# gruai/koifish

Measured on AMD Instinct MI355X. Metric: tokens/sec/GPU Qwen3 4-bit prefill+decode; achieved HBM GB/s vs peak, higher is better.
Workload: dtype u4 weights x bf16, fp32 accumulate

## Files before the change

koifish_amd/csrc/kf_abi.hip:

```cpp
#include <stdarg.h>
#include <stdio.h>
#include <string.h>


#include <mutex>
#include <math.h>
#include <stdlib.h>

#include <vector>

#include "kf_gemm_plan.h"

struct kf_ctx {
    int device;
    hipStream_t stream;
    bool own_stream;
    bool capturing;
    float* amax_val;
    int* amax_idx;
    int canonical;
    void* scratch;
    size_t scratch_bytes;
    struct DeqCopy {
        const void* key[3];
// ... 1246 lines not shown
    if (rc != KF_OK) return fail(rc, "kf_xengine_check: HIP failure");
    if (err) return fail(KF_INTERNAL_ERR, "kf_xengine: error word 0x%x (8: an XCD did not get 32 workgroups; 64: a position beyond the cache rows (TP form); others: a hand-off poll timed out -- the launch was not fully resident)", err);
    return KF_OK;
}
int kf_xengine_reset(kf_ctx* c, kf_xengine* e) {
    CHKCTX(c);
    if (!e || !e->h) return fail(KF_INVALID_ARGS, "kf_xengine_reset: null engine");
    if (c->capturing) return fail(KF_INVALID_ARGS, "kf_xengine_reset: not while capturing");
    if (hipStreamSynchronize(c->stream) != hipSuccess) return fail(KF_HIP_CHECK, "kf_xengine_reset: HIP failure");
    const int rc = kf::xengine_reset(e->h, c->stream);
    if (rc != KF_OK) return fail(rc, "kf_xengine_reset: HIP failure");
    return KF_OK;
}
int kf_xengine_destroy(kf_xengine* e) {
    if (e) {
        kf::xengine_free(e->h);
        delete e;
    }
    return KF_OK;
}
int kfdbg_xengine_variant(kf_xengine* e, int nwv, int depth) { return (e && e->h) ? kf::xengine_set_variant(e->h, nwv, depth) : -1; }
int kfdbg_xengine_form(int shape_class, int fmt, int n_seq, int n_layer, int stamps, int two_wpc, int* out) {
    const kf::XForm* f = kf::xengine_form(shape_class, fmt, n_seq, n_layer, stamps != 0, two_wpc != 0);
    if (!f || !out) return -1;
    out[0] = f->nwv, out[1] = f->depth, out[2] = f->wpc, out[3] = f->nb, out[4] = f->dbg;
    return 0;
}
int kfdbg_engine_form(int shape_class, int fmt, int canon, int stamps, int n_layer, int* out) {
    const kf::EngForm* f = kf::engine_form(shape_class, fmt, canon != 0, stamps != 0, n_layer);
    if (!f || !out) return -1;
    out[0] = f->shape_class, out[1] = f->fmt, out[2] = f->canon, out[3] = f->dbg, out[4] = (int)f->smem(n_layer);
    return 0;
}
int kfdbg_xengine_stamps_enable(kf_xengine* e, int seq, int wg, int max_steps) { return (e && e->h) ? kf::xengine_debug_enable(e->h, seq, wg, max_steps) : -1; }
int kfdbg_xengine_stamps(kf_xengine* e, unsigned long long* h_out, int n_words) { return (e && e->h) ? kf::xengine_debug_read(e->h, h_out, n_words) : -1; }
int kfdbg_engine_stamps_enable(kf_engine* e, int wg) { return (e && e->h) ? kf::engine_debug_enable(e->h, wg) : -1; }
int kfdbg_engine_stamps(kf_engine* e, unsigned long long* h_out, int n_words) { return (e && e->h) ? kf::engine_debug_read(e->h, h_out, n_words) : -1; }
int kfdbg_engine_set_delays(kf_engine* e, const int* d6) {
    if (!e || !e->h || !d6) return -1;
    kf::engine_set_delays(e->h, d6);
    return 0;
}
int kfdbg_gemm_plan(const kf::GemmProblem* P, kf::GemmPlan* out) {
    if (!P || !out) return -1;
    *out = kf::gemm_plan(*P);
    return 0;
}
int kfdbg_set_knob(const char* name, long value) {
    if (!name) return -1;
    kf::Knobs& k = kf::g_knobs;
    if (!strcmp(name, "q4_perm")) k.q4_perm = (int)value;
    else if (!strcmp(name, "q2_tab")) k.q2_tab = (int)value;
    else if (!strcmp(name, "q1_tab")) k.q1_tab = (int)value;
    else if (!strcmp(name, "gemv_waves")) k.gemv_waves = value;
    else if (!strcmp(name, "gemv_stream")) k.gemv_stream = (int)value;
    else if (!strcmp(name, "gemv_xf2")) k.gemv_xf2 = (int)value;
    else if (!strcmp(name, "attn_gq_split")) k.attn_gq_split = (int)value;
    else if (!strcmp(name, "attn_pair_min")) k.attn_pair_min = (int)value;
    else return -1;
    return 0;
}
int kf_engine_destroy(kf_engine* e) {
    if (e) {
        kf::engine_free(e->h);
        delete e;
    }
// ... 5 lines not shown
```

koifish_amd/csrc/kf_engine.hip:

```cpp
#include <stdlib.h>
#include <string.h>

#include <vector>

#include <type_traits>

#include "kf_engine_common.h"

namespace kf {


struct EngXOff {
    int xA, qkv, ao, xB, act, part, hbest, tokg, end;
};
constexpr EngXOff eng_xoff(int dim, int qd, int kvd, int ffn, int hd) {
    EngXOff o{};
    o.xA = 0, o.qkv = o.xA + eng_gran_dw(dim), o.ao = o.qkv + eng_gran_dw(qd + 2 * kvd), o.xB = o.ao + eng_gran_dw(qd), o.act = o.xB + eng_gran_dw(dim);
    o.part = o.act + eng_gran_dw(ffn);
    o.hbest = o.part + eng_gran_dw(2 * (qd / hd) * KF_ATTN_MAX_SPLITS * (2 * hd + 4));
    o.tokg = o.hbest + eng_gran_dw(2 * ENG_NWG);
    o.end = o.tokg + eng_gran_dw(2);
    return o;
}
constexpr int eng_lq_stride(int gq, int hd) { return ((gq * hd + 2 * hd) * 4 + 255) / 256 * 64; }
constexpr int eng_lp_stride(int gq, int hd) { return (gq * KF_ATTN_MAX_SPLITS * (2 * hd + 4) * 8 + 255) / 256 * 32; }
constexpr size_t eng_loc_bytes(int gq, int hd) { return 1024 + (size_t)8 * eng_lq_stride(gq, hd) * 4 + (size_t)8 * eng_lp_stride(gq, hd) * 8; }

struct EngArgs {
    const EngLayer* layers;
    int n_layer;
    int n_steps;
    float eps, qk_eps;
    const float* rope_table;
    const int32_t* d_state;
    const uint16_t* x_in;
    const uint16_t* emb;
    const int32_t* d_forced;
    int emb_rows;
    uint16_t* x_out;
    uint32_t* xch;
    int* ws;
    char* loc;
    int nsp, chunk, merge_e;
    int kv_stride;
    int max_seq;
    float qbias[7];
    int delay[6];
    g_u32x4 head_w;
    g_u16 head_norm;
    uint16_t* logits;
    int32_t* d_state_w;
// ... 20 lines not shown
        for (int i = 0; i < NR; i++) {
            const int r = wave + i * NWV;
            g[i] = __builtin_bit_cast(u32x4, __builtin_amdgcn_raw_buffer_load_b128(rs, ((r < NLD ? r : wave) * 64 + lane) * 16, 0, 16 ));
        }
#pragma unroll
        for (int i = 0; i < NR; i++) bad = (wave + i * NWV < NLD) ? tags_bad(g[i], tagw, bad) : bad;
        if (wave >= NLD || all_good(bad)) {
            if (nsweeps) *nsweeps = spins + 1;
            break;
        }
        if (dead || spins > ENG_SPIN_MAX) {
            if (!dead && lane == 0) atomicOr(ws + 1, 1);
            dead = true;
            break;
        }
        __builtin_amdgcn_s_sleep(1);
    }
#pragma unroll
    for (int i = 0; i < NR; i++) {
        const int r = wave + i * NWV;
        if (r >= NLD) continue;
        const int e0 = 4 * (r * 64 + lane);
        const uint32_t o0 = (g[i].x & 0xffffu) | (g[i].y << 16), o1 = (g[i].z & 0xffffu) | (g[i].w << 16);
        if (F32X) {
            const int q = e0 >> 2, c = q / XCH, j = q - c * XCH;
            xs[j * NBLK + c] = u32x4{o0 << 16, o0 & 0xffff0000u, o1 << 16, o1 & 0xffff0000u};
        } else {
            const int q = e0 >> 3, c = q / XCH, j = q - c * XCH;
            reinterpret_cast<u32x2*>(xs + j * NBLK + c)[(e0 >> 2) & 1] = u32x2{o0, o1};
        }
    }
}

template <bool PAIRED, int MAXS>
struct MvRegs {
    u32x4 w[MAXS], w2[PAIRED ? MAXS : 1];
    uint16_t st[MAXS], ze[MAXS], st2[PAIRED ? MAXS : 1], ze2[PAIRED ? MAXS : 1];
};
template <class PL, int NCW>
constexpr int c_maxs() { return ((PL::spg + NCW - 1) / NCW) * PL::iters; }
template <class PL, int NCW>
__device__ __forceinline__ MvAt mv_at(int k, int s0, int cw, int lane, int Mj) {
    const int sub = lane >> PL::lpr_log2, ll = lane & (PL::LPR - 1);
    const int sl = k / PL::iters, it = k - sl * PL::iters;
    const int s_loc = cw + sl * NCW;
    MvAt q;
    q.row = (s0 + s_loc) * PL::RPS + sub;
    q.col = it * PL::LPR + ll;
    q.ok = s_loc < PL::spg && q.row < Mj && q.col < PL::nBlk;
    return q;
}
template <class PL, int NCW, int FMT, int MAXS>
__device__ __forceinline__ void mv_prefetch(const EngMat m, const EngMat m2, int s0, int cw, int lane, int Mj, MvRegs<PL::PAIRED, MAXS>& R, uint32_t hotbits = 0xffffffffu) {
    constexpr bool GAMA = BlockDot<FMT>::HAS_GAMA;
    constexpr int gshift = FMT >= FMT_Q4 ? (FMT == FMT_Q4 || FMT == FMT_Q4P || FMT == FMT_Q1T || FMT == FMT_Q2T ? 2 : (FMT == FMT_Q2 ? 1 : 0)) : 0;
#pragma unroll
    for (int k = 0; k < MAXS; k++) {
        const MvAt q = mv_at<PL, NCW>(k, s0, cw, lane, Mj);
        int row = q.row < Mj ? q.row : Mj - 1;
        row = row > 0 ? row : 0;
        row = ((hotbits >> ((q.row - s0 * PL::RPS) & 31)) & 1u) ? row : 0;
        const int col = q.col < PL::nBlk ? q.col : PL::nBlk - 1;
        const uint32_t bidx = (uint32_t)row * (uint32_t)PL::nBlk + (uint32_t)col;
        if constexpr (FMT == FMT_Q1T) {
            const uint32_t di = (bidx & ~3u) + (3u - (bidx & 3u));
            R.w[k] = u32x4{__builtin_nontemporal_load(reinterpret_cast<const uint32_t KF_GLOBAL*>(m.w) + di), 0u, 0u, 0u};
// ... 120 lines not shown
    double* comb;
    uint32_t* outb;
    int* cnt;
    double* msc;
    int* pub;
    const u32x4* q1tab;
    const uint32_t* hotbits;
};
struct EngSlice {
    int pos, len, nsp, kvh, split, h0, t0, t1, me0;
    bool has_unit, empty, own_new, has_merge;
    int xcc, rank;
    int j1;
    int s1;
    int M1;
    int q_out0;
};

__device__ __forceinline__ void wg_publish(const EngLds& L, int phase, uint32_t* buf, int idx0, int nrows, int nwaves, int lane, bool local = false) {
    int old = 0;
    if (lane == 0) old = __hip_atomic_fetch_add(L.cnt, 1, __ATOMIC_RELAXED, __HIP_MEMORY_SCOPE_WORKGROUP);
    old = __builtin_amdgcn_readfirstlane(old);
    if (old != nwaves - 1) return;
    if (lane == 0) *L.cnt = 0;
    if (4 * lane < nrows) {
        const u32x4 v = *reinterpret_cast<const u32x4*>(L.outb + 4 * lane);
        if (local)
            *reinterpret_cast<u32x4*>(buf + idx0 + 4 * lane) = v;
        else
            __builtin_amdgcn_raw_buffer_store_b128(v, eng_rsrc(buf + idx0, (uint32_t)nrows * 4u), lane * 16, 0, 16 );
    }
    if (lane == 0) __hip_atomic_fetch_add(L.pub + phase, 1, __ATOMIC_RELAXED, __HIP_MEMORY_SCOPE_WORKGROUP);
}

template <int FMT_, int GQ_, int HD_, int NWV_, int DIM_, int QD_, int KVD_, int FFN_, int NWG_, bool XMAP_, bool DBG_, bool CANON_ = true>
struct EngCfg {
    static constexpr int FMT = FMT_, GQ = GQ_, HD = HD_, NWV = NWV_, DIM = DIM_, QD = QD_, KVD = KVD_, FFN = FFN_, NWG = NWG_;
    static constexpr bool XMAP = XMAP_, DBG = DBG_;
    static constexpr int AHR = DIM_ > 1024 ? ENG_AH_REGS_WIDE : ENG_AH_REGS;
    static constexpr int AHR_P = DIM_ > 1024 ? ENG_AH_PAIR_WIDE : ENG_AH_REGS;
    static constexpr bool CANON = CANON_;
    static_assert(FMT_ == FMT_Q4 || FMT_ == FMT_Q4P || FMT_ == FMT_Q1T || FMT_ == FMT_Q2T, "storages with a BlockPrep: 32-weight blocks dequantised ahead of the hand-off (16 pair words each)");
    static constexpr bool F32X = CANON_;
    static constexpr int XCH = F32X ? 8 : 4;
    static constexpr int n_head = QD_ / HD_, n_kv = KVD_ / HD_;
    using SH = EngShape<FMT_, DIM_, QD_, KVD_, FFN_, NWG_>;
    static constexpr int xA = eng_xoff(DIM_, QD_, KVD_, FFN_, HD_).xA, qkv = eng_xoff(DIM_, QD_, KVD_, FFN_, HD_).qkv, ao = eng_xoff(DIM_, QD_, KVD_, FFN_, HD_).ao,
                         xB = eng_xoff(DIM_, QD_, KVD_, FFN_, HD_).xB, act = eng_xoff(DIM_, QD_, KVD_, FFN_, HD_).act, part = eng_xoff(DIM_, QD_, KVD_, FFN_, HD_).part,
                         hbest = eng_xoff(DIM_, QD_, KVD_, FFN_, HD_).hbest, tokg = eng_xoff(DIM_, QD_, KVD_, FFN_, HD_).tokg;
    static constexpr int HnBlk = DIM_ / 8, Hlpr_log2 = c_lpr_log2(DIM_ / 8, 1L << 20), HLPR = 1 << Hlpr_log2, HRPS = 64 >> Hlpr_log2, Hiters = (HnBlk + HLPR - 1) / HLPR;
    static constexpr int lq_stride = eng_lq_stride(GQ_, HD_), lp_stride = eng_lp_stride(GQ_, HD_);
    static constexpr int ME = pow2_ceil((QD_ + NWG_ - 1) / NWG_), PSH = KF_ATTN_MAX_SPLITS * (2 * HD_ + 4), NLM = (KF_ATTN_MAX_SPLITS * ME * 2 + 127) / 128;
    static_assert(ME <= 64 && ME <= HD_, "merge elements per workgroup");
};
template <class C>
__device__ __forceinline__ uint32_t* eng_lqkv(const EngArgs& a, int xcc) { return reinterpret_cast<uint32_t*>(a.loc + 1024) + (size_t)xcc * C::lq_stride; }
template <class C>
__device__ __forceinline__ unsigned long long* eng_lpart(const EngArgs& a, int xcc) {
    return reinterpret_cast<unsigned long long*>(a.loc + 1024 + (size_t)8 * C::lq_stride * 4) + (size_t)xcc * C::lp_stride;
}

template <class C>
struct EngAttnState {
    static constexpr int U = 2;
    u32x4 kk[U], vv[U];
    uint16_t nw0, nw1;
    float rc, rs;
};
template <class C>
__device__ __forceinline__ void eng_attn_rope(const EngArgs& a, const EngSlice& S, int lane, EngAttnState<C>& T) {
    T.rc = 1.f, T.rs = 0.f;
    if (a.rope_table && lane < (C::HD >> 1)) {
        const float* tab_pos = a.rope_table + (size_t)S.pos * C::HD;
        T.rc = tab_pos[2 * lane], T.rs = tab_pos[2 * lane + 1];
    }
}
template <class C>
__device__ __forceinline__ void eng_attn_normw(const EngLayer& ly, int wave, int lane, EngAttnState<C>& T) {
    const int half = C::HD >> 1, j = lane < half ? lane : half - 1;
    static_assert(C::GQ < C::NWV, "the q heads and the new key are prepared by different waves");
    g_u16 np = wave < C::GQ ? ly.norm_q : ly.norm_k;
    T.nw0 = T.nw1 = 0;
// ... 142 lines not shown
                    st_gran64(dst + oi, gen, __uint_as_float((uint32_t)ob)), st_gran64(dst + oi + 1, gen, __uint_as_float((uint32_t)(ob >> 32)));
                    if (d == 0) st_gran64(dst + mi, gen, ms), st_gran64(dst + mi + 1, gen, __uint_as_float((uint32_t)lb)), st_gran64(dst + mi + 2, gen, __uint_as_float((uint32_t)(lb >> 32)));
                }
            }
        }
    } else if (nsp > 1) {
        for (int i = tid; i < GQ * hd; i += NWA * 64) {
            const int hq = i >> hd_log2, d = i & (hd - 1);
            constexpr int ME = C::ME, MAXSP = KF_ATTN_MAX_SPLITS;
            const size_t oi = ((size_t)(d / ME) * (MAXSP * ME) + (size_t)S.split * ME + (d & (ME - 1))) * 2, mi = (size_t)hd * MAXSP * 2 + (size_t)S.split * 4;
            const unsigned long long gg = (unsigned long long)gen << 32;
            if (XMAP) {
                unsigned long long* dst = eng_lpart<C>(a, S.xcc) + (size_t)hq * C::PSH;
                dst[oi] = gg, dst[oi + 1] = gg;
                if (d == 0) dst[mi] = gg | 0xff800000u, dst[mi + 1] = gg, dst[mi + 2] = gg;
            } else {
                unsigned long long* dst = reinterpret_cast<unsigned long long*>(a.xch + C::part) + (size_t)(h0 + hq) * C::PSH;
                st_gran64(dst + oi, gen, 0.f), st_gran64(dst + oi + 1, gen, 0.f);
                if (d == 0) st_gran64(dst + mi, gen, -__builtin_inff()), st_gran64(dst + mi + 1, gen, 0.f), st_gran64(dst + mi + 2, gen, 0.f);
            }
        }
    }
}

template <class C>
__device__ __forceinline__ void eng_poller_main(const EngArgs& a, const EngLds& L, const EngSlice& S, int epoch, int step, int wg, int lane) {
    using SH = typename C::SH;
    using P1 = typename SH::P1;
    using P4 = typename SH::P4;
    using P5 = typename SH::P5;
    using P6 = typename SH::P6;
    constexpr int FMT = C::FMT, GQ = C::GQ, HD = C::HD, NWV = C::NWV;
    constexpr bool XMAP = C::XMAP, DBG = C::DBG;
    constexpr int ND = C::DIM / 256, NQD = C::QD / 256, NF = C::FFN / 256;
    constexpr int XCH = C::XCH, hd = HD, hd_log2 = HD == 128 ? 7 : 6;
    bool dead = false;
    const bool has1 = XMAP ? true : wg * P1::spg < P1::total, has4 = wg * P4::spg < P4::total, has5 = wg * P5::spg < P5::total, has6 = wg * P6::spg < P6::total;
    constexpr int NCW1 = ENG_P1_SHARE ? NWV : NWV - 1, S1 = c_maxs<P1, NCW1>(), NWP1 = P1::spg < NCW1 ? P1::spg : NCW1;
    constexpr bool P1_SHARE = ENG_P1_SHARE && P1::spg >= NWV;
    const float qb1 = S.j1 == 0 ? a.qbias[0] : (S.j1 == 1 ? a.qbias[1] : a.qbias[2]);
    const int row0_1 = S.s1 * P1::RPS;
    MvRegs<false, S1> r1;
    auto mat1 = [&](int l) {
        return L.lay[l].m[S.j1];
    };
    if (P1_SHARE) mv_prefetch<P1, NCW1, FMT, S1>(mat1(0), mat1(0), S.s1, NWV - 1, lane, S.M1, r1);
    EngAttnState<C> T;
#pragma unroll
    for (int u = 0; u < EngAttnState<C>::U; u++) T.kk[u] = T.vv[u] = u32x4{0, 0, 0, 0};
    eng_attn_rope<C>(a, S, lane, T);
    if (S.has_unit && !S.empty) eng_attn_issue<C>(a, L.lay[0], S, NWV - 1, lane, T, 0);
    int sw[4] = {0, 0, 0, 0};
    int swt[6] = {0, 0, 0, 0, 0, 0};
    for (int l = 0; l < a.n_layer; l++) {
        const EngLayer& ly = L.lay[l];
        const uint32_t gen = (uint32_t)epoch * (uint32_t)a.n_layer + (uint32_t)l, tag = gen & 0xffffu;
        if (S.has_unit && !S.empty) eng_attn_normw<C>(ly, NWV - 1, lane, T);
        MvPhase<C, P1, NCW1, S1> w1;
        if (P1_SHARE) w1.ahead(qb1, 0.f, NWV - 1, lane, r1, L.q1tab);
        ENG_STAMP(0, 0);
        if (has1 || has4) {
            if (l == 0) {
                const uint16_t* x0 = a.x_in;
                if (!x0) {
                    int tok = a.d_state[0];
                    if (step > 0) {
                        const __amdgpu_buffer_rsrc_t rt = eng_rsrc(a.xch + C::tokg, 8u);
// ... 145 lines not shown
                    for (int k = 0; k < MAXSP; k++) o += ldexp_d(mv[k], shl[k]);
                }
            }
            const uint32_t gr = (tag << 16) | (uint32_t)f2bf((float)(o / Lt));
            const bool holder = (4 * ME <= 64) ? ((lane & 3) == 0 && (lane >> 2) < ME) : (lane < ME);
            const int he = (4 * ME <= 64) ? (lane >> 2) : lane;
            uint32_t* const ao_dst = a.xch + C::ao + (XMAP ? S.h0 * hd : 0) + S.me0;
            if (ME >= 4) {
                uint32_t* mo = reinterpret_cast<uint32_t*>(L.msc + ME * MAXSP);
                if (holder) mo[he] = gr;
                if (4 * lane < ME) __builtin_amdgcn_raw_buffer_store_b128(*reinterpret_cast<const u32x4*>(mo + 4 * lane), eng_rsrc(ao_dst, (uint32_t)ME * 4u), lane * 16, 0, 16 );
            } else if (holder) {
                __hip_atomic_store(ao_dst + he, gr, __ATOMIC_RELAXED, __HIP_MEMORY_SCOPE_AGENT);
            }
        }
        ENG_STAMP(0, 4);
        if (ENG_COOP) {
            if (has4) eng_wait_pub(nullptr, 0, a.delay[3], dead);
            __syncthreads();
            if (has4) eng_poll_stage_part<XCH, NQD, P4::nBlk, NWV, C::F32X>(a.xch + C::ao, tag, L.xs[1], NWV - 1, lane, a.ws, dead, &sw[1]);
        } else if (has4) {
            eng_poll_stage<XCH, NQD, P4::nBlk, false, false, C::F32X>(a.xch + C::ao, nullptr, tag, nullptr, 0.f, L.xs[1], nullptr, lane, a.ws, dead, &sw[1], nullptr, 0, a.delay[3]);
        }
        ENG_STAMP(0, 5);
        __syncthreads();
        if (has5 || has6)
            eng_poll_stage<XCH, ND, P5::nBlk, true, false, C::F32X>(a.xch + C::xB, nullptr, tag, ly.norm_post, a.eps, L.xs[0], L.xrawB, lane, a.ws, dead, &sw[2], has4 ? L.pub + 1 : nullptr, l + 1,
                                                           a.delay[4]);
        ENG_STAMP(0, 6);
        __syncthreads();
        if (ENG_COOP) {
            if (has6) eng_wait_pub(has5 ? L.pub + 2 : nullptr, l + 1, a.delay[5], dead);
            __syncthreads();
            if (has6) eng_poll_stage_part<XCH, NF, P6::nBlk, NWV, C::F32X>(a.xch + C::act, tag, L.xs[1], NWV - 1, lane, a.ws, dead, &sw[3]);
        } else if (has6) {
            eng_poll_stage<XCH, NF, P6::nBlk, false, false, C::F32X>(a.xch + C::act, nullptr, tag, nullptr, 0.f, L.xs[1], nullptr, lane, a.ws, dead, &sw[3], has5 ? L.pub + 2 : nullptr, l + 1, a.delay[5]);
        }
        ENG_STAMP(0, 7);
        swt[0] += sw[0], swt[3] += sw[1], swt[4] += sw[2], swt[5] += sw[3];
        if (DBG && wg == a.dbg_wg && lane == 0)
            a.dbg[((size_t)l * 2) * 16 + 8] = (unsigned long long)sw[0] | ((unsigned long long)sw[1] << 16) | ((unsigned long long)sw[2] << 32) | ((unsigned long long)sw[3] << 48);
        __syncthreads();
    }
    if (wg == 0 && lane == 0) {
#pragma unroll
        for (int i = 0; i < 6; i++) atomicAdd(a.ws + 8 + i, swt[i]);
        atomicAdd(a.ws + 14, a.n_layer);
    }
}

template <class C>
__device__ __forceinline__ void eng_compute_main(const EngArgs& a, const EngLds& L, const EngSlice& S, int epoch, int wg, int wave, int lane) {
    using SH = typename C::SH;
    using P1 = typename SH::P1;
    using P4 = typename SH::P4;
    using P5 = typename SH::P5;
    using P6 = typename SH::P6;
    constexpr int FMT = C::FMT, NWV = C::NWV;
    constexpr bool XMAP = C::XMAP, DBG = C::DBG;
    constexpr int NCW = NWV - 1;
    constexpr int NCW1 = ENG_P1_SHARE ? NWV : NWV - 1;
    constexpr int S1 = c_maxs<P1, NCW1>(), S4 = c_maxs<P4, NCW>(), S5 = c_maxs<P5, NCW>(), S6 = c_maxs<P6, NCW>();
    static_assert(P1::R % 4 == 0 && P4::R % 4 == 0 && P5::R % 4 == 0 && P6::R % 4 == 0 && P1::R <= 64 && P4::R <= 64 && P5::R <= 64 && P6::R <= 64, "rows per workgroup");
    static_assert(P1::total % P1::spg == 0 && P4::total % P4::spg == 0 && P5::total % P5::spg == 0 && P6::total % P6::spg == 0, "whole workgroups");
    static_assert(P1::S1 % P1::spg == 0 && P1::S2 % P1::spg == 0, "a workgroup's P1 rows belong to one matrix");
    constexpr int NWP1 = P1::spg < NCW1 ? P1::spg : NCW1, NWP4 = P4::spg < NCW ? P4::spg : NCW, NWP5 = P5::spg < NCW ? P5::spg : NCW, NWP6 = P6::spg < NCW ? P6::spg : NCW;
    const bool has1 = XMAP ? true : wg * P1::spg < P1::total, has4 = wg * P4::spg < P4::total, has5 = wg * P5::spg < P5::total, has6 = wg * P6::spg < P6::total;
    const float qb1 = S.j1 == 0 ? a.qbias[0] : (S.j1 == 1 ? a.qbias[1] : a.qbias[2]);
    const int row0_1 = S.s1 * P1::RPS;
// ... 41 lines not shown
            const int lane_a = lane + lz;
            eng_attn_phase<C>(a, L, S, ly, gen, tag, wave, lane_a, T, l, wg);
            if (wave == 0) ENG_STAMP(1, 3);
            if (DBG && wave == 0) {
                asm volatile("s_waitcnt vmcnt(0)" ::: "memory");
                ENG_STAMP(1, 10);
            }
            if (!S.empty) eng_attn_issue<C>(a, L.lay[ln], S, wave, lane_a, T, 0);
        }

        MvPhase<C, P4, NCW, S4> w4;
        w4.ahead(a.qbias[3], 0.f, wave, lane_m, r4, L.q1tab);
        if (ENG_COOP) {
            __syncthreads();
            if (has4) eng_poll_stage_part<C::XCH, C::QD / 256, P4::nBlk, NWV, C::F32X>(a.xch + C::ao, tag, L.xs[1], wave, lane_m, a.ws, dead);
        }
        __syncthreads();
        if (wave == 0) ENG_STAMP(1, 4);
        const uint32_t hot5 = L.hotbits[l];
        mv_prefetch<P5, NCW, FMT, S5>(ly.m[4], ly.m[5], wg * P5::spg, wave, lane_m, P5::M0, r5, hot5);
        w4.run(wg * P4::spg, wave, lane_m, P4::M0, L.xs[1], 0xffffffffu, r4, [&](int row, float v, float) {
            const uint16_t o = f2bf(v);
            L.outb[row - wg * P4::R] = (tag << 16) | (uint32_t)f2bf(bf2f(L.xrawA[row]) + bf2f(o));
        });
        if (has4 && wave < NWP4) wg_publish(L, 1, a.xch + C::xB, wg * P4::R, P4::R, NWP4, lane_m);
        if (wave == 0) ENG_STAMP(1, 5);
        MvPhase<C, P5, NCW, S5> w5;
        w5.ahead(a.qbias[4], a.qbias[5], wave, lane_m, r5, L.q1tab);
        __syncthreads();
        if (wave == 0) ENG_STAMP(1, 6);
        mv_prefetch<P6, NCW, FMT, S6>(ly.m[6], ly.m[6], wg * P6::spg, wave, lane_m, P6::M0, r6);
        w5.run(wg * P5::spg, wave, lane_m, P5::M0, L.xs[0], L.hotbits[l], r5, [&](int row, float v, float v2) {
            const float gt = round_bf16(v), up = round_bf16(v2);
            L.outb[row - wg * P5::R] = (tag << 16) | (uint32_t)f2bf((gt * up) / (1.0f + kf_expf(-gt)));
        });
        if (has5 && wave < NWP5) wg_publish(L, 2, a.xch + C::act, wg * P5::R, P5::R, NWP5, lane_m);
        if (wave == 0) ENG_STAMP(1, 7);
        MvPhase<C, P6, NCW, S6> w6;
        w6.ahead(a.qbias[6], 0.f, wave, lane_m, r6, L.q1tab);
        if (ENG_COOP) {
            __syncthreads();
            if (has6) eng_poll_stage_part<C::XCH, C::FFN / 256, P6::nBlk, NWV, C::F32X>(a.xch + C::act, tag, L.xs[1], wave, lane_m, a.ws, dead);
        }
        __syncthreads();
        if (wave == 0) ENG_STAMP(1, 8);
        mv_prefetch<P1, NCW1, FMT, S1>(mat1(ln), mat1(ln), S.s1, wave, lane_m, S.M1, r1);
        w6.run(wg * P6::spg, wave, lane_m, P6::M0, L.xs[1], 0xffffffffu, r6, [&](int row, float v, float) {
            const uint16_t o = f2bf(v);
            const uint16_t y = f2bf(bf2f(L.xrawB[row]) + bf2f(o));
            if (last) a.x_out[row] = y;
            L.outb[row - wg * P6::R] = (tag_next << 16) | (uint32_t)y;
        });
        if ((!last || a.head_on) && has6 && wave < NWP6) wg_publish(L, 3, a.xch + C::xA, wg * P6::R, P6::R, NWP6, lane_m);
        if (wave == 0) ENG_STAMP(1, 9);
    }
}


template <class C>
__device__ __forceinline__ void eng_head_main(const EngArgs& a, const EngLds& L, int epoch, bool more_steps, int wg, int wave, int lane) {
    constexpr int NWV = C::NWV, NWG = C::NWG, nBlk = C::HnBlk, LPR = C::HLPR, RPS = C::HRPS, ITERS = C::Hiters, HG = 4;
    constexpr int ND = C::DIM / 256;
    const int sub = lane >> C::Hlpr_log2, ll = lane & (LPR - 1);
    const int total = (a.vocab + RPS - 1) / RPS, spg = (total + NWG - 1) / NWG;
    const int s_wg = wg * spg;
    int s_end = s_wg + spg;
    s_end = s_end < total ? s_end : total;
    const int nmine = s_end > s_wg + wave ? (s_end - s_wg - wave + NWV - 1) / NWV : 0;
    const int nbatch = (nmine + HG - 1) / HG;
    u32x4 w[2][HG][ITERS];
    auto issue = [&](int b, int buf) {
#pragma unroll
        for (int g = 0; g < HG; g++) {
            int i = b * HG + g;
            i = i < nmine ? i : (nmine > 0 ? nmine - 1 : 0);
// ... 319 lines not shown
using EC2 = EngCfg<FMT, 2, 64, ENG_NWV, 256, 256, 128, 512, ENG_NWG, false, DBG, CANON>;
template <int FMT, bool DBG, bool CANON>
using EC3 = EngCfg<FMT, 2, 128, ENG_NWV, 2048, 2048, 1024, 6144, ENG_NWG, true, DBG, CANON>;

struct EngShapeRow {
    int sc, hd, dim, q_dim, kv_dim, ffn;
};
template <class C>
constexpr EngShapeRow eng_shape(int sc) {
    return EngShapeRow{sc, C::HD, C::DIM, C::QD, C::KVD, C::FFN};
}
static const EngShapeRow eng_shapes[] = {eng_shape<EC1<FMT_Q4P, false, true>>(1), eng_shape<EC2<FMT_Q4P, false, true>>(2), eng_shape<EC3<FMT_Q4P, false, true>>(3)};
static const EngShapeRow* eng_shape_of(const kf_engine_desc* d) {
    for (const EngShapeRow& s : eng_shapes)
        if (d->head_dim == s.hd && d->dim == s.dim && d->n_head * d->head_dim == s.q_dim && d->n_kv * d->head_dim == s.kv_dim && d->ffn == s.ffn) return &s;
    return nullptr;
}

#define ENG_ORDERS(EC, FMT, DBG, sc) eng_form<EC<FMT, DBG, true>>(sc), eng_form<EC<FMT, DBG, false>>(sc)
static const EngForm eng_forms[] = {ENG_ORDERS(EC1, FMT_Q4P, false, 1), ENG_ORDERS(EC1, FMT_Q4P, true, 1), ENG_ORDERS(EC1, FMT_Q1T, false, 1), ENG_ORDERS(EC1, FMT_Q2T, false, 1),
                                    ENG_ORDERS(EC2, FMT_Q4P, false, 2), ENG_ORDERS(EC2, FMT_Q1T, false, 2), ENG_ORDERS(EC2, FMT_Q2T, false, 2),
                                    ENG_ORDERS(EC3, FMT_Q4P, false, 3)};
#undef ENG_ORDERS
const EngForm* engine_form(int sc, int fmt, bool canon, bool stamps, int n_layer) {
    auto find = [&](bool dbg) -> const EngForm* {
        for (const EngForm& f : eng_forms)
            if (f.shape_class == sc && f.fmt == fmt && f.canon == canon && f.dbg == dbg) return &f;
        return nullptr;
    };
    const EngForm* f = stamps ? find(true) : nullptr;
    if (!f) f = find(false);
    return f && f->smem(n_layer) <= 160 * 1024 ? f : nullptr;
}
static bool eng_plans_match(const EngForm* f, const kf_engine_desc* d) {
    const int q_dim = d->n_head * d->head_dim, kv_dim = d->n_kv * d->head_dim;
    const int K[4] = {d->dim, q_dim, d->dim, d->ffn}, M[4][3] = {{q_dim, kv_dim, kv_dim}, {d->dim, 0, 0}, {d->ffn, d->ffn, 0}, {d->dim, 0, 0}};
    const long rows[4] = {(long)q_dim + 2 * kv_dim, d->dim, d->ffn, d->dim};
    for (int i = 0; i < 4; i++) {
        const CPlan& p = f->plan[i];
        if (p.K != K[i] || p.nBlk != K[i] / 32 || p.lpr_log2 != gemv_lpr_log2(p.nBlk, rows[i])) return false;
        for (int j = 0; j < 3; j++)
            if (p.M[j] != M[i][j]) return false;
    }
    return true;
}

int eng_fill_layers(const kf_engine_desc* d, EngLayer* tab, float* qbias, bool qbias_set, bool& q4p_ok, int* fmt_io, bool allow_hot) {
    const int hd = d->head_dim, q_dim = d->n_head * hd, kv_dim = d->n_kv * hd;
    const int Ks[7] = {d->dim, d->dim, d->dim, q_dim, d->dim, d->dim, d->ffn}, Ms[7] = {q_dim, kv_dim, kv_dim, d->dim, d->ffn, d->ffn, d->dim};
    for (int l = 0; l < d->n_layer; l++) {
        const kf_engine_layer& Ly = d->layers[l];
        if (Ly.hot_ffn && !allow_hot) return KF_UNSUPPORTED_DATATYPE;
        if (!Ly.norm_in || !Ly.norm_post || !Ly.kcache || !Ly.vcache || (((uintptr_t)Ly.kcache | (uintptr_t)Ly.vcache) & 15) != 0) return KF_UNSUPPORTED_DATATYPE;
        for (int j = 0; j < 7; j++) {
            const kf_weight& w = Ly.w[j];
            const int wf = gemv_fmt_of(&w), ef = wf == FMT_Q4 ? FMT_Q4P : (wf == FMT_Q1 ? FMT_Q1T : (wf == FMT_Q2 ? FMT_Q2T : -1));
            if (ef < 0 || (!fmt_io && ef != FMT_Q4P) || (fmt_io && *fmt_io != 0 && *fmt_io != ef)) return KF_UNSUPPORTED_DATATYPE;
            if (fmt_io) *fmt_io = ef;
            if (w.ne0 != Ms[j] || w.ne1 != Ks[j] || w.qzeros || w.qscales || !w.gama || w.lGroup != 128 || (Ks[j] % 128) != 0 || ((uintptr_t)w.data & 15) != 0)
                return KF_UNSUPPORTED_DATATYPE;
            const long rows = j < 3 ? (long)q_dim + 2 * kv_dim : (j == 4 || j == 5 ? (long)d->ffn : (long)Ms[j]);
            if (gemv_lpr_log2(Ks[j] / 32, rows) < 2) q4p_ok = false;
            tab[l].m[j].w = (g_u32x4)(uintptr_t)w.data;
            tab[l].m[j].zero = (g_u16)(uintptr_t)(w.gama + w.ne0 + w.ne1);
            tab[l].m[j].step = (g_u16)(uintptr_t)(w.gama + w.ne0 + w.ne1 + (size_t)w.ne0 * w.ne1 / w.lGroup);
            if (l == 0 && !qbias_set) qbias[j] = (float)w.qBias;
// ... 270 lines not shown
```

koifish_amd/csrc/kf_kernels.h:

```cpp
#pragma once
#include "../../include/kf_abi.h"
#include "kf_device.h"

namespace kf {

enum {
    FMT_BF16 = 0, FMT_F8 = 1, FMT_Q4 = 2, FMT_Q2 = 3, FMT_Q1 = 4,
    FMT_Q4P = 5,
    FMT_Q4R = 6,
    FMT_Q1T = 7,
    FMT_Q2T = 8
};
inline bool is_row_lut(const kf_weight* w) { return w->quant != KF_QUANT_GROUP; }
enum { GEMV_PLAIN = 0, GEMV_PAIRED = 1, GEMV_ARGMAX = 2 };
constexpr int KF_MAX_ARGMAX_PARTIALS = 4096;
constexpr int KF_ATTN_MAX_SPLITS = 32;
constexpr int KF_ATTN_CNT_BYTES = 16384;

struct GemvJob {
    const void* w;
    const uint16_t* zero;
    const uint16_t* step;
    uint16_t* y;
    long long y_pos_stride;
// ... 78 lines not shown
};
int attn_launch(hipStream_t st, AttnArgs& a);
int attn_splits(int pos_bound, int n_kv);
int attn_prefill_mfma_launch(hipStream_t st, const uint16_t* q, const uint16_t* kc, const uint16_t* vc, uint16_t* out, int pos0, int n_tok, long long q_stride,
                             int n_head, int n_kv, int hd, int kv_stride, int n_seq = 1, long long out_stride = 0 );
int qknorm_rope_launch(hipStream_t st, uint16_t* q, uint16_t* k, const uint16_t* wq, const uint16_t* wk, const float* table, int pos,
                       const int* d_pos, int n_head, int n_kv, int hd, float eps, int n_tok = 1, long long q_stride = 0, long long k_stride = 0, int seq_len = 0,
                       float* rstd_q = nullptr, float* rstd_k = nullptr);

struct Knobs {
    int q4_perm = 1;
    int q2_tab = 1;
    int attn_pair_min = 256;
    int attn_gq_split = 4;
    int q1_tab = 1;
    long gemv_waves = 0;
    int gemv_stream = 1;
    int gemv_xf2 = 1;
};
extern Knobs g_knobs;
struct EngineHost;
struct CPlan {
    int K, nBlk, lpr_log2, iters, njobs, M[3], slot0[3], total, spg;
};
struct EngForm {
    int shape_class, fmt;
    bool canon, dbg;
    CPlan plan[4];
    size_t (*smem)(int n_layer);
    int (*go)(EngineHost* E, hipStream_t st);
};
const EngForm* engine_form(int shape_class, int fmt, bool canon, bool stamps, int n_layer);
size_t engine_ws_bytes(const kf_engine_desc* d);
int engine_build(const kf_engine_desc* d, void* ws, size_t ws_bytes, hipStream_t st, EngineHost** out, const char** why = nullptr, bool dry = false);
int engine_tune(EngineHost* E, hipStream_t st, uint16_t* x_out, const int32_t* d_state, int pos_bound, int passes, float* us_before, float* us_after);
int engine_stats(EngineHost* E, hipStream_t st, int pos_bound, int* out14);
int engine_step(EngineHost* E, hipStream_t st, const uint16_t* x_in, uint16_t* x_out, const int32_t* d_state, int pos_bound, int with_head = 0, int n_steps = 1);
int engine_set_head(EngineHost* E, const kf_weight* w, const uint16_t* norm_w, uint16_t* logits, int32_t* d_tokens_out);
int engine_set_embedding(EngineHost* E, const kf_weight* w, const int32_t* d_forced);
int engine_error_word(EngineHost* E, hipStream_t st, int* h_err);
void engine_set_canonical(EngineHost* E, int on);
int engine_reset(EngineHost* E, hipStream_t st);
void engine_free(EngineHost* E);
int engine_debug_read(EngineHost* E, unsigned long long* h_out, int n_words);
int engine_debug_enable(EngineHost* E, int wg);
void engine_set_delays(EngineHost* E, const int* d6);

struct XEngineHost;
struct XForm {
    int shape_class, fmt;
    int nwv, depth, wpc, nb;
    bool dbg;
    size_t (*smem)(int n_layer);
    int (*go)(XEngineHost* E, hipStream_t st);
};
const XForm* xengine_form(int shape_class, int fmt, int n_seq, int n_layer, bool stamps, bool two_wpc);
size_t xengine_ws_bytes(const kf_engine_desc* d);
int xengine_build(const kf_engine_desc* d, int n_seq, long long kv_seq_stride, void* ws, size_t ws_bytes, hipStream_t st, XEngineHost** out, const char** why = nullptr, bool dry = false);
int xengine_steps(XEngineHost* E, hipStream_t st, int32_t* d_state, uint16_t* x_out, int with_head, int n_steps);
size_t xengine_ws_bytes_tp(const kf_engine_desc* rank0);
int xengine_build_tp(const kf_engine_desc* const* ranks, int world, void* ws, size_t ws_bytes, hipStream_t st, XEngineHost** out, const char** why = nullptr);
int xengine_set_head_tp(XEngineHost* E, const kf_weight* const* shards, const int* row0, const uint16_t* norm_w, uint16_t* logits, int32_t* d_tokens_out, int tokens_stride);
int xengine_set_embedding(XEngineHost* E, const kf_weight* w, const int32_t* d_forced, int forced_stride);
int xengine_set_head(XEngineHost* E, const kf_weight* w, const uint16_t* norm_w, uint16_t* logits, int32_t* d_tokens_out, int tokens_stride);
int xengine_error_word(XEngineHost* E, hipStream_t st, int* h_err);
int xengine_reset(XEngineHost* E, hipStream_t st);
// ... 52 lines not shown
```

Measured before the change: 2323.

## Pack FFN activation hand-off densely: three bf16 values plus tag per 64-bit granule

```diff
diff --git a/koifish_amd/csrc/kf_abi.hip b/koifish_amd/csrc/kf_abi.hip
--- a/koifish_amd/csrc/kf_abi.hip
+++ b/koifish_amd/csrc/kf_abi.hip
@@ -1302,6 +1302,7 @@
     out[0] = f->shape_class, out[1] = f->fmt, out[2] = f->canon, out[3] = f->dbg, out[4] = (int)f->smem(n_layer);
     return 0;
 }
+int kfdbg_engine_xlayout(int shape_class, int* out16) { return out16 ? kf::engine_xlayout(shape_class, out16) : -1; }
 int kfdbg_xengine_stamps_enable(kf_xengine* e, int seq, int wg, int max_steps) { return (e && e->h) ? kf::xengine_debug_enable(e->h, seq, wg, max_steps) : -1; }
 int kfdbg_xengine_stamps(kf_xengine* e, unsigned long long* h_out, int n_words) { return (e && e->h) ? kf::xengine_debug_read(e->h, h_out, n_words) : -1; }
 int kfdbg_engine_stamps_enable(kf_engine* e, int wg) { return (e && e->h) ? kf::engine_debug_enable(e->h, wg) : -1; }
diff --git a/koifish_amd/csrc/kf_engine.hip b/koifish_amd/csrc/kf_engine.hip
--- a/koifish_amd/csrc/kf_engine.hip
+++ b/koifish_amd/csrc/kf_engine.hip
@@ -10,13 +10,22 @@
 namespace kf {
 
 
+struct EngDense {
+    int R, G, nwg, ng;
+};
+constexpr EngDense eng_dense(int dim, int ffn) {
+    const CPlan p = c_plan(dim, 32, ffn, ffn, 0, true, ENG_NWG);
+    EngDense d{};
+    d.R = p.spg * (64 >> p.lpr_log2), d.G = (d.R + 2) / 3, d.nwg = (p.total + p.spg - 1) / p.spg, d.ng = d.nwg * d.G;
+    return d;
+}
 struct EngXOff {
     int xA, qkv, ao, xB, act, part, hbest, tokg, end;
 };
 constexpr EngXOff eng_xoff(int dim, int qd, int kvd, int ffn, int hd) {
     EngXOff o{};
     o.xA = 0, o.qkv = o.xA + eng_gran_dw(dim), o.ao = o.qkv + eng_gran_dw(qd + 2 * kvd), o.xB = o.ao + eng_gran_dw(qd), o.act = o.xB + eng_gran_dw(dim);
-    o.part = o.act + eng_gran_dw(ffn);
+    o.part = o.act + eng_gran_dw(2 * eng_dense(dim, ffn).ng);
     o.hbest = o.part + eng_gran_dw(2 * (qd / hd) * KF_ATTN_MAX_SPLITS * (2 * hd + 4));
     o.tokg = o.hbest + eng_gran_dw(2 * ENG_NWG);
     o.end = o.tokg + eng_gran_dw(2);
@@ -103,6 +112,87 @@
     }
 }
 
+template <bool F32X, int XCH, int NBLK>
+__device__ __forceinline__ void eng_stage_pair(u32x4* xs, int e, uint32_t lo, uint32_t hi) {
+    if (F32X) {
+        const int q = e >> 2, c = q / XCH, j = q - c * XCH;
+        reinterpret_cast<u32x2*>(xs + j * NBLK + c)[(e >> 1) & 1] = u32x2{lo << 16, hi << 16};
+    } else {
+        const int q = e >> 3, c = q / XCH, j = q - c * XCH;
+        reinterpret_cast<uint32_t*>(xs + j * NBLK + c)[(e >> 1) & 3] = (lo & 0xffffu) | (hi << 16);
+    }
+}
+template <bool F32X, int XCH, int NBLK>
+__device__ __forceinline__ void eng_stage_one(u32x4* xs, int e, uint32_t v) {
+    if (F32X) {
+        const int q = e >> 2, c = q / XCH, j = q - c * XCH;
+        reinterpret_cast<uint32_t*>(xs + j * NBLK + c)[e & 3] = v << 16;
+    } else {
+        const int q = e >> 3, c = q / XCH, j = q - c * XCH;
+        reinterpret_cast<uint16_t*>(xs + j * NBLK + c)[e & 7] = (uint16_t)v;
+    }
+}
+template <int XCH, int NBLK, int R, int G, int NG, int NWV, bool F32X = true>
+__device__ __forceinline__ void eng_poll_stage_dense(const uint32_t* gsrc, uint32_t tag, u32x4* xs, int wave, int lane, int* ws, bool& dead, int* nsweeps = nullptr) {
+    constexpr int NLD = (NG + 127) / 128, NR = (NLD + NWV - 1) / NWV;
+    constexpr bool WHOLE = NG % 128 == 0, EXACT = 3 * G == R;
+    const __amdgpu_buffer_rsrc_t rs = eng_rsrc(gsrc, (uint32_t)NG * 8u);
+    const uint32_t tagw = tag << 16;
+    u32x4 g[NR];
+    for (int spins = 0;; spins++) {
+        uint32_t bad = 0;
+#pragma unroll
+        for (int i = 0; i < NR; i++) {
+            const int r = wave + i * NWV;
+            g[i] = __builtin_bit_cast(u32x4, __builtin_amdgcn_raw_buffer_load_b128(rs, ((r < NLD ? r : wave) * 64 + lane) * 16, 0, 16 ));
+        }
+#pragma unroll
+        for (int i = 0; i < NR; i++) {
+            const int r = wave + i * NWV, gi = 2 * (r * 64 + lane);
+            if (r >= NLD) continue;
+            bad |= (WHOLE || gi < NG) ? (g[i].y ^ tagw) & 0xffff0000u : 0u;
+            bad |= (WHOLE || gi + 1 < NG) ? (g[i].w ^ tagw) & 0xffff0000u : 0u;
+        }
+        if (wave >= NLD || all_good(bad)) {
+            if (nsweeps) *nsweeps = spins + 1;
+            break;
+        }
+        if (dead || spins > ENG_SPIN_MAX) {
+            if (!dead && lane == 0) atomicOr(ws + 1, 1);
+            dead = true;
+            break;
+        }
+        __builtin_amdgcn_s_sleep(KF_SWEEP_SLEEP);
+    }
+#pragma unroll
+    for (int i = 0; i < NR; i++) {
+        const int r = wave + i * NWV, gi = 2 * (r * 64 + lane);
+        if (r >= NLD) continue;
+        const uint32_t v[6] = {g[i].x & 0xffffu, g[i].x >> 16, g[i].y & 0xffffu, g[i].z & 0xffffu, g[i].z >> 16, g[i].w & 0xffffu};
+        if constexpr (EXACT) {
+            if (WHOLE || gi < NG) {
+                const int e = 3 * gi;
+                eng_stage_pair<F32X, XCH, NBLK>(xs, e, v[0], v[1]);
+                if (WHOLE || gi + 1 < NG) {
+                    eng_stage_pair<F32X, XCH, NBLK>(xs, e + 2, v[2], v[3]);
+                    eng_stage_pair<F32X, XCH, NBLK>(xs, e + 4, v[4], v[5]);
+                } else {
+                    eng_stage_one<F32X, XCH, NBLK>(xs, e + 2, v[2]);
+                }
+            }
+        } else {
+#pragma unroll
+            for (int h = 0; h < 2; h++) {
+                const int gh = gi + h, w = gh / G, k = gh - w * G;
+                if (gh >= NG) continue;
+#pragma unroll
+                for (int s = 0; s < 3; s++)
+                    if (3 * k + s < R) eng_stage_one<F32X, XCH, NBLK>(xs, w * R + 3 * k + s, v[3 * h + s]);
+            }
+        }
+    }
+}
+
 template <bool PAIRED, int MAXS>
 struct MvRegs {
     u32x4 w[MAXS], w2[PAIRED ? MAXS : 1];
@@ -289,6 +379,23 @@
     }
     if (lane == 0) __hip_atomic_fetch_add(L.pub + phase, 1, __ATOMIC_RELAXED, __HIP_MEMORY_SCOPE_WORKGROUP);
 }
+__device__ __forceinline__ int eng_dense_slot(int r) { return (r / 3) * 4 + (r - (r / 3) * 3); }
+template <int R, int G>
+__device__ __forceinline__ void wg_publish_dense(const EngLds& L, int phase, uint32_t* buf, int g0, uint32_t tag, int nwaves, int lane) {
+    static_assert(G <= 32, "a workgroup's granules in outb");
+    int old = 0;
+    if (lane == 0) old = __hip_atomic_fetch_add(L.cnt, 1, __ATOMIC_RELAXED, __HIP_MEMORY_SCOPE_WORKGROUP);
+    old = __builtin_amdgcn_readfirstlane(old);
+    if (old != nwaves - 1) return;
+    if (lane == 0) *L.cnt = 0;
+    if (lane < G) {
+        u32x2 v = reinterpret_cast<const u32x2*>(L.outb)[lane];
+        if (3 * lane + 1 >= R) v.x &= 0xffffu;
+        v.y = (3 * lane + 2 < R ? (v.y & 0xffffu) : 0u) | (tag << 16);
+        __builtin_amdgcn_raw_buffer_store_b64(v, eng_rsrc(buf + 2 * g0, (uint32_t)G * 8u), lane * 8, 0, 16 );
+    }
+    if (lane == 0) __hip_atomic_fetch_add(L.pub + phase, 1, __ATOMIC_RELAXED, __HIP_MEMORY_SCOPE_WORKGROUP);
+}
 
 template <int FMT_, int GQ_, int HD_, int NWV_, int DIM_, int QD_, int KVD_, int FFN_, int NWG_, bool XMAP_, bool DBG_, bool CANON_ = true>
 struct EngCfg {
@@ -305,6 +412,8 @@
     static constexpr int xA = eng_xoff(DIM_, QD_, KVD_, FFN_, HD_).xA, qkv = eng_xoff(DIM_, QD_, KVD_, FFN_, HD_).qkv, ao = eng_xoff(DIM_, QD_, KVD_, FFN_, HD_).ao,
                          xB = eng_xoff(DIM_, QD_, KVD_, FFN_, HD_).xB, act = eng_xoff(DIM_, QD_, KVD_, FFN_, HD_).act, part = eng_xoff(DIM_, QD_, KVD_, FFN_, HD_).part,
                          hbest = eng_xoff(DIM_, QD_, KVD_, FFN_, HD_).hbest, tokg = eng_xoff(DIM_, QD_, KVD_, FFN_, HD_).tokg;
+    static constexpr int actR = eng_dense(DIM_, FFN_).R, actG = eng_dense(DIM_, FFN_).G, actNG = eng_dense(DIM_, FFN_).ng;
+    static_assert(actR == SH::P5::R && actNG == (SH::P5::total / SH::P5::spg) * actG, "EngDense is the gate | up plan");
     static constexpr int HnBlk = DIM_ / 8, Hlpr_log2 = c_lpr_log2(DIM_ / 8, 1L << 20), HLPR = 1 << Hlpr_log2, HRPS = 64 >> Hlpr_log2, Hiters = (HnBlk + HLPR - 1) / HLPR;
     static constexpr int lq_stride = eng_lq_stride(GQ_, HD_), lp_stride = eng_lp_stride(GQ_, HD_);
     static constexpr int ME = pow2_ceil((QD_ + NWG_ - 1) / NWG_), PSH = KF_ATTN_MAX_SPLITS * (2 * HD_ + 4), NLM = (KF_ATTN_MAX_SPLITS * ME * 2 + 127) / 128;
@@ -513,7 +622,7 @@
     using P6 = typename SH::P6;
     constexpr int FMT = C::FMT, GQ = C::GQ, HD = C::HD, NWV = C::NWV;
     constexpr bool XMAP = C::XMAP, DBG = C::DBG;
-    constexpr int ND = C::DIM / 256, NQD = C::QD / 256, NF = C::FFN / 256;
+    constexpr int ND = C::DIM / 256, NQD = C::QD / 256;
     constexpr int XCH = C::XCH, hd = HD, hd_log2 = HD == 128 ? 7 : 6;
     bool dead = false;
     const bool has1 = XMAP ? true : wg * P1::spg < P1::total, has4 = wg * P4::spg < P4::total, has5 = wg * P5::spg < P5::total, has6 = wg * P6::spg < P6::total;
@@ -725,9 +834,10 @@
         if (ENG_COOP) {
             if (has6) eng_wait_pub(has5 ? L.pub + 2 : nullptr, l + 1, a.delay[5], dead);
             __syncthreads();
-            if (has6) eng_poll_stage_part<XCH, NF, P6::nBlk, NWV, C::F32X>(a.xch + C::act, tag, L.xs[1], NWV - 1, lane, a.ws, dead, &sw[3]);
+            if (has6) eng_poll_stage_dense<XCH, P6::nBlk, C::actR, C::actG, C::actNG, NWV, C::F32X>(a.xch + C::act, tag, L.xs[1], NWV - 1, lane, a.ws, dead, &sw[3]);
         } else if (has6) {
-            eng_poll_stage<XCH, NF, P6::nBlk, false, false, C::F32X>(a.xch + C::act, nullptr, tag, nullptr, 0.f, L.xs[1], nullptr, lane, a.ws, dead, &sw[3], has5 ? L.pub + 2 : nullptr, l + 1, a.delay[5]);
+            eng_wait_pub(has5 ? L.pub + 2 : nullptr, l + 1, a.delay[5], dead);
+            eng_poll_stage_dense<XCH, P6::nBlk, C::actR, C::actG, C::actNG, 1, C::F32X>(a.xch + C::act, tag, L.xs[1], 0, lane, a.ws, dead, &sw[3]);
         }
         ENG_STAMP(0, 7);
         swt[0] += sw[0], swt[3] += sw[1], swt[4] += sw[2], swt[5] += sw[3];
@@ -835,15 +945,15 @@
         mv_prefetch<P6, NCW, FMT, S6>(ly.m[6], ly.m[6], wg * P6::spg, wave, lane_m, P6::M0, r6);
         w5.run(wg * P5::spg, wave, lane_m, P5::M0, L.xs[0], L.hotbits[l], r5, [&](int row, float v, float v2) {
             const float gt = round_bf16(v), up = round_bf16(v2);
-            L.outb[row - wg * P5::R] = (tag << 16) | (uint32_t)f2bf((gt * up) / (1.0f + kf_expf(-gt)));
+            reinterpret_cast<uint16_t*>(L.outb)[eng_dense_slot(row - wg * P5::R)] = f2bf((gt * up) / (1.0f + kf_expf(-gt)));
         });
-        if (has5 && wave < NWP5) wg_publish(L, 2, a.xch + C::act, wg * P5::R, P5::R, NWP5, lane_m);
+        if (has5 && wave < NWP5) wg_publish_dense<C::actR, C::actG>(L, 2, a.xch + C::act, wg * C::actG, tag, NWP5, lane_m);
         if (wave == 0) ENG_STAMP(1, 7);
         MvPhase<C, P6, NCW, S6> w6;
         w6.ahead(a.qbias[6], 0.f, wave, lane_m, r6, L.q1tab);
         if (ENG_COOP) {
             __syncthreads();
-            if (has6) eng_poll_stage_part<C::XCH, C::FFN / 256, P6::nBlk, NWV, C::F32X>(a.xch + C::act, tag, L.xs[1], wave, lane_m, a.ws, dead);
+            if (has6) eng_poll_stage_dense<C::XCH, P6::nBlk, C::actR, C::actG, C::actNG, NWV, C::F32X>(a.xch + C::act, tag, L.xs[1], wave, lane_m, a.ws, dead);
         }
         __syncthreads();
         if (wave == 0) ENG_STAMP(1, 8);
@@ -1229,6 +1339,23 @@
     if (!f) f = find(false);
     return f && f->smem(n_layer) <= 160 * 1024 ? f : nullptr;
 }
+int engine_xlayout(int sc, int* out) {
+    for (const EngShapeRow& s : eng_shapes) {
+        if (s.sc != sc) continue;
+        const EngXOff o = eng_xoff(s.dim, s.q_dim, s.kv_dim, s.ffn, s.hd);
+        const EngDense d = eng_dense(s.dim, s.ffn);
+        const int v[16] = {o.xA, o.qkv, o.ao, o.xB, o.act, o.part, o.hbest, o.tokg, o.end, d.R, d.G, d.nwg, d.ng, 0, 0, 0};
+        for (int i = 0; i < 16; i++) out[i] = v[i];
+        for (const EngForm& f : eng_forms)
+            if (f.shape_class == sc) {
+                const CPlan& p = f.plan[2];
+                out[13] = p.spg * (64 >> p.lpr_log2), out[14] = (p.total + p.spg - 1) / p.spg, out[15] = p.M[0];
+                break;
+            }
+        return 0;
+    }
+    return -1;
+}
 static bool eng_plans_match(const EngForm* f, const kf_engine_desc* d) {
     const int q_dim = d->n_head * d->head_dim, kv_dim = d->n_kv * d->head_dim;
     const int K[4] = {d->dim, q_dim, d->dim, d->ffn}, M[4][3] = {{q_dim, kv_dim, kv_dim}, {d->dim, 0, 0}, {d->ffn, d->ffn, 0}, {d->dim, 0, 0}};
diff --git a/koifish_amd/csrc/kf_kernels.h b/koifish_amd/csrc/kf_kernels.h
--- a/koifish_amd/csrc/kf_kernels.h
+++ b/koifish_amd/csrc/kf_kernels.h
@@ -134,6 +134,7 @@
 };
 const EngForm* engine_form(int shape_class, int fmt, bool canon, bool stamps, int n_layer);
 size_t engine_ws_bytes(const kf_engine_desc* d);
+int engine_xlayout(int shape_class, int* out16);
 int engine_build(const kf_engine_desc* d, void* ws, size_t ws_bytes, hipStream_t st, EngineHost** out, const char** why = nullptr, bool dry = false);
 int engine_tune(EngineHost* E, hipStream_t st, uint16_t* x_out, const int32_t* d_state, int pos_bound, int passes, float* us_before, float* us_after);
 int engine_stats(EngineHost* E, hipStream_t st, int pos_bound, int* out14);
```

Result: no change. 2338, median of 6 (+0.6%).
